# kason-huang/StreamVLN

Hardware: AMD Instinct MI355X
Metric: action-steps/sec (8-frame window, StreamVLN-Qwen-1.5) (higher is better)
Workload: dtype bf16

## Files before the change

### streamvln_amd/csrc/gemv.hip

```cpp
#include <hip/hip_ext.h>

#include <cstdlib>
#include <stdexcept>

#include "common.h"
#include "kernels.h"

namespace svln {

namespace {

typedef __attribute__((ext_vector_type(2))) __bf16 bf16x2_t;
typedef float f32x2 __attribute__((ext_vector_type(2)));
constexpr int GEMV_THREADS = 256;
constexpr int GEMV_WAVES = GEMV_THREADS / 64;


template <typename T> struct WPlain {
    using X = T;
    static constexpr int EPC = Elt<T>::PER_CHUNK;
    struct Row { const T* w; };
    using Chunk = uint4;
    using Acc = float;
    static constexpr bool X_LATE = false;
    static constexpr int ROWS_GRID_CAP = 0;
    static constexpr int KS_R = 2;
    static constexpr int KS_KW_NARROW = 4;
    static constexpr bool KS_PAIRED = true;
    SVLN_DEV static Row row(const GemvArgs& p, size_t n) { return {(const T*)p.W + n * p.ldw}; }
    SVLN_DEV static Chunk load(const Row& r, int ci) { return load_nt(r.w + (size_t)ci * EPC); }
    SVLN_DEV static Acc zero() { return 0.0f; }
    SVLN_DEV static void fma(const Chunk& w, const f32x2* x2, Acc& acc) {
        float f[EPC];
        chunk_to_f32<T>(w, f);
#pragma unroll
        for (int e = 0; e < EPC; ++e) acc = fmaf(f[e], x2[e / 2][e % 2], acc);
    }
    SVLN_DEV static float sum(Acc a) { return a; }
    SVLN_DEV static float row_scale(const GemvArgs&, size_t) { return 1.0f; }
};

struct WPacked {
    using X = bf16;
    using Acc = f32x2;
    SVLN_DEV static Acc zero() { return f32x2{0.0f, 0.0f}; }
    SVLN_DEV static float sum(Acc a) { return a[0] + a[1]; }
};

struct WE4m3 : WPacked {
    static constexpr int EPC = 16;
    struct Row { const uint8_t* w; };
    using Chunk = uint4;
    static constexpr bool X_LATE = false;
    static constexpr int ROWS_GRID_CAP = 0;
    static constexpr int KS_R = 4;
    static constexpr int KS_KW_NARROW = 4;
    static constexpr bool KS_PAIRED = false;
    SVLN_DEV static Row row(const GemvArgs& p, size_t n) { return {(const uint8_t*)p.w8 + n * p.ldw}; }
    SVLN_DEV static Chunk load(const Row& r, int ci) { return load_nt(r.w + (size_t)ci * 16); }
    SVLN_DEV static void fma(const Chunk& w, const f32x2* x2, Acc& acc) {
        const unsigned d[4] = {w.x, w.y, w.z, w.w};
#pragma unroll
        for (int q = 0; q < 4; ++q) {
            const f32x2 lo = __builtin_amdgcn_cvt_pk_f32_fp8((int)d[q], false);
            const f32x2 hi = __builtin_amdgcn_cvt_pk_f32_fp8((int)d[q], true);
            acc = __builtin_elementwise_fma(lo, x2[2 * q], acc);
            acc = __builtin_elementwise_fma(hi, x2[2 * q + 1], acc);
        }
    }
    SVLN_DEV static float row_scale(const GemvArgs& p, size_t n) { return p.scale[n]; }
};

struct WMxfp4 : WPacked {
    static constexpr int EPC = 32;
    struct Row { const uint8_t* q; const uint8_t* s; };
    struct Chunk { uint4 q; unsigned s; };
    static constexpr bool X_LATE = true;
    static constexpr int ROWS_GRID_CAP = 0;
    static constexpr int KS_R = 4;
    static constexpr int KS_KW_NARROW = 2;
    static constexpr bool KS_PAIRED = false;
    SVLN_DEV static Row row(const GemvArgs& p, size_t n) {
        return {(const uint8_t*)p.w4 + n * ((size_t)p.ldw / 2), p.e8 + n * ((size_t)p.ldw / 32)};
    }
    SVLN_DEV static Chunk load(const Row& r, int ci) { return {load_nt(r.q + (size_t)ci * 16), r.s[ci]}; }
    SVLN_DEV static void fma(const Chunk& w, const f32x2* x2, Acc& acc) {
        const unsigned d[4] = {w.q.x, w.q.y, w.q.z, w.q.w};
        const float sc = __uint_as_float(w.s << 23);
#pragma unroll
        for (int q = 0; q < 4; ++q) {
            acc = __builtin_elementwise_fma((f32x2)__builtin_amdgcn_cvt_scalef32_pk_f32_fp4(d[q], sc, 0), x2[4 * q], acc);
            acc = __builtin_elementwise_fma((f32x2)__builtin_amdgcn_cvt_scalef32_pk_f32_fp4(d[q], sc, 1), x2[4 * q + 1], acc);
            acc = __builtin_elementwise_fma((f32x2)__builtin_amdgcn_cvt_scalef32_pk_f32_fp4(d[q], sc, 2), x2[4 * q + 2], acc);
            acc = __builtin_elementwise_fma((f32x2)__builtin_amdgcn_cvt_scalef32_pk_f32_fp4(d[q], sc, 3), x2[4 * q + 3], acc);
        }
    }
    SVLN_DEV static float row_scale(const GemvArgs&, size_t) { return 1.0f; }
};

SVLN_DEV void p12_high_bytes(unsigned c, unsigned t0, unsigned t1, unsigned& ha, unsigned& hb) {
    ha = __builtin_amdgcn_perm(t1, t0, c & 0x07070707u) | ((c << 4) & 0x80808080u);
    hb = __builtin_amdgcn_perm(t1, t0, (c >> 4) & 0x07070707u) | (c & 0x80808080u);
}
SVLN_DEV uint4 p12_decode(unsigned lo0, unsigned lo1, unsigned c, unsigned t0, unsigned t1) {
    unsigned ha, hb;
    p12_high_bytes(c, t0, t1, ha, hb);
    return make_uint4(__builtin_amdgcn_perm(ha, lo0, 0x05010400u), __builtin_amdgcn_perm(ha, lo0, 0x07030602u),
                      __builtin_amdgcn_perm(hb, lo1, 0x05010400u), __builtin_amdgcn_perm(hb, lo1, 0x07030602u));
}
SVLN_DEV void p12_decode_f32(unsigned lo0, unsigned lo1, unsigned c, unsigned t0, unsigned t1, float* f) {
    unsigned ha, hb;
    p12_high_bytes(c, t0, t1, ha, hb);
    f[0] = __uint_as_float(__builtin_amdgcn_perm(ha, lo0, 0x04000C0Cu)); f[1] = __uint_as_float(__builtin_amdgcn_perm(ha, lo0, 0x05010C0Cu));
    f[2] = __uint_as_float(__builtin_amdgcn_perm(ha, lo0, 0x06020C0Cu)); f[3] = __uint_as_float(__builtin_amdgcn_perm(ha, lo0, 0x07030C0Cu));
    f[4] = __uint_as_float(__builtin_amdgcn_perm(hb, lo1, 0x04000C0Cu)); f[5] = __uint_as_float(__builtin_amdgcn_perm(hb, lo1, 0x05010C0Cu));
    f[6] = __uint_as_float(__builtin_amdgcn_perm(hb, lo1, 0x06020C0Cu)); f[7] = __uint_as_float(__builtin_amdgcn_perm(hb, lo1, 0x07030C0Cu));
}
typedef __attribute__((ext_vector_type(2))) unsigned int u32x2;
struct WP12 {
    using X = bf16;
    static constexpr int EPC = 8;
    struct Row { const uint8_t* pk; const bf16* w; unsigned t0, t1, m0, m1; };
    struct Chunk { u32x2 a, b; unsigned t0, t1; bool fb, odd; };
    using Acc = float;
    static constexpr bool X_LATE = false;
    static constexpr int ROWS_GRID_CAP = 1024;
    static constexpr int KS_R = 2;
    static constexpr int KS_KW_NARROW = 4;
    static constexpr bool KS_PAIRED = true;
    SVLN_DEV static size_t uniform(size_t v) {
        const unsigned lo = (unsigned)__builtin_amdgcn_readfirstlane((int)(unsigned)v), hi = (unsigned)__builtin_amdgcn_readfirstlane((int)(unsigned)(v >> 32));
        return ((size_t)hi << 32) | lo;
    }
    SVLN_DEV static Row row(const GemvArgs& p, size_t n) {
        const uint4 rec = *(const uint4*)((const uint8_t*)p.prec + n * 16);
        return {(const uint8_t*)p.wp + uniform(n * p12_row_bytes(p.K)), (const bf16*)p.W + uniform(n * (size_t)p.ldw),
                (unsigned)__builtin_amdgcn_readfirstlane((int)rec.x), (unsigned)__builtin_amdgcn_readfirstlane((int)rec.y),
                (unsigned)__builtin_amdgcn_readfirstlane((int)rec.z), (unsigned)__builtin_amdgcn_readfirstlane((int)rec.w)};
    }
    SVLN_DEV static Chunk load(const Row& r, int ci) {
        const int blk = __builtin_amdgcn_readfirstlane(ci >> 6);
        const unsigned l = (unsigned)ci & 63u;
        Chunk c; c.t0 = r.t0; c.t1 = r.t1; c.odd = l & 1u;
        c.fb = (((blk & 32) ? r.m1 : r.m0) >> (blk & 31)) & 1u;
        const uint8_t* wb = (const uint8_t*)r.w + (size_t)blk * 1024;
        const uint8_t* pb = r.pk + (size_t)blk * 768;
        c.a = __builtin_nontemporal_load((const u32x2*)((c.fb ? wb : pb) + (l << (c.fb ? 4 : 3))));
        c.b = __builtin_nontemporal_load((const u32x2*)((c.fb ? wb + 8 : pb + 512) + (c.fb ? l << 4 : (l >> 1) << 3)));
        return c;
    }
    SVLN_DEV static Acc zero() { return 0.0f; }
    SVLN_DEV static void fma(const Chunk& w, const f32x2* x2, Acc& acc) {
        float f[EPC];
        if (w.fb) chunk_to_f32<bf16>(make_uint4(w.a.x, w.a.y, w.b.x, w.b.y), f);
        else p12_decode_f32(w.a.x, w.a.y, w.odd ? w.b.y : w.b.x, w.t0, w.t1, f);
#pragma unroll
        for (int e = 0; e < EPC; ++e) acc = fmaf(f[e], x2[e / 2][e % 2], acc);
    }
    SVLN_DEV static float sum(Acc a) { return a; }
    SVLN_DEV static float row_scale(const GemvArgs&, size_t) { return 1.0f; }
};

template <typename X, int PLANES>
SVLN_DEV float stage_x(float* xs, const GemvArgs& p, int nch) {
    constexpr int XEPC = Elt<X>::PER_CHUNK;
    constexpr int XP = XEPC / 4, XPW = PLANES / XP;
    __shared__ float red[GEMV_WAVES];
    const X* x = (const X*)p.x;
    const X* g = (const X*)p.norm_w;
    const int tid = threadIdx.x, nxch = p.K / XEPC;
    float ss = 0.0f;
    for (int ci = tid; ci < nxch; ci += GEMV_THREADS) {
        float f[XEPC];
        chunk_to_f32<X>(*(const uint4*)(x + (size_t)ci * XEPC), f);
        if (g) {
            float gf[XEPC];
            chunk_to_f32<X>(*(const uint4*)(g + (size_t)ci * XEPC), gf);
#pragma unroll
            for (int e = 0; e < XEPC; ++e) { ss = fmaf(f[e], f[e], ss); f[e] *= gf[e]; }
        }
        const int cj = ci / XPW, p0 = (ci % XPW) * XP;
#pragma unroll
        for (int q = 0; q < XP; ++q)
            *(float4*)(xs + (size_t)(p0 + q) * nch * 4 + (size_t)cj * 4) = make_float4(f[4 * q], f[4 * q + 1], f[4 * q + 2], f[4 * q + 3]);
    }
    if (g) {
        ss = wave_sum(ss);
        if ((tid & 63) == 0) red[tid >> 6] = ss;
    }
    __syncthreads();
    if (!g) return 1.0f;
    float tot = 0.0f;
#pragma unroll
    for (int w = 0; w < GEMV_WAVES; ++w) tot += red[w];
    return rsqrtf(tot / (float)p.K + p.eps);
}

template <int PLANES>
SVLN_DEV void load_x(const float* xs, int nch, int ci, f32x2* x2) {
#pragma unroll
    for (int q = 0; q < PLANES; ++q) {
        const float4 v = *(const float4*)(xs + (size_t)q * nch * 4 + (size_t)ci * 4);
        x2[2 * q] = f32x2{v.x, v.y};
        x2[2 * q + 1] = f32x2{v.z, v.w};
    }
}
template <typename P, bool NORM>
SVLN_DEV float load_xg(const typename P::X* xg, const typename P::X* gg, int ci, f32x2* x2, float ss) {
    using X = typename P::X;
    constexpr int XEPC = Elt<X>::PER_CHUNK;
#pragma unroll
    for (int h = 0; h < P::EPC / XEPC; ++h) {
        float fh[XEPC];
        chunk_to_f32<X>(*(const uint4*)(xg + (size_t)ci * P::EPC + h * XEPC), fh);
        if (NORM) {
            float gf[XEPC];
            chunk_to_f32<X>(*(const uint4*)(gg + (size_t)ci * P::EPC + h * XEPC), gf);
#pragma unroll
            for (int e = 0; e < XEPC; ++e) { ss = fmaf(fh[e], fh[e], ss); fh[e] *= gf[e]; }
        }
#pragma unroll
        for (int e = 0; e < XEPC / 2; ++e) x2[h * (XEPC / 2) + e] = f32x2{fh[2 * e], fh[2 * e + 1]};
    }
    return ss;
}

template <typename P, int R, bool XLDS>
SVLN_DEV void dot_accum(const typename P::Row (&rows)[R], const float* xs, const typename P::X* xg, int nch, int c0, int cstep, int lane,
                        typename P::Acc (&acc)[R]) {
    constexpr int EPC = P::EPC;
    auto get_x = [&](int ci, f32x2* x2) {
        if (XLDS) load_x<EPC / 4>(xs, nch, ci, x2);
        else load_xg<P, false>(xg, nullptr, ci, x2, 0.0f);
    };
    const int stride = 64 * cstep;
    int ci = c0 + lane;
    for (; ci + stride < nch; ci += 2 * stride) {
        typename P::Chunk w0[R], w1[R];
#pragma unroll
        for (int r = 0; r < R; ++r) {
            w0[r] = P::load(rows[r], ci);
            w1[r] = P::load(rows[r], ci + stride);
        }
        f32x2 x0[EPC / 2];
        get_x(ci, x0);
        if (P::X_LATE) {
#pragma unroll
            for (int r = 0; r < R; ++r) P::fma(w0[r], x0, acc[r]);
            get_x(ci + stride, x0);
#pragma unroll
            for (int r = 0; r < R; ++r) P::fma(w1[r], x0, acc[r]);
        } else {
            f32x2 x1[EPC / 2];
            get_x(ci + stride, x1);
#pragma unroll
            for (int r = 0; r < R; ++r) {
                P::fma(w0[r], x0, acc[r]);
                P::fma(w1[r], x1, acc[r]);
            }
        }
    }
    for (; ci < nch; ci += stride) {
        typename P::Chunk w0[R];
#pragma unroll
        for (int r = 0; r < R; ++r) w0[r] = P::load(rows[r], ci);
        f32x2 x0[EPC / 2];
        get_x(ci, x0);
#pragma unroll
        for (int r = 0; r < R; ++r) P::fma(w0[r], x0, acc[r]);
    }
}

template <typename X>
SVLN_DEV void store_out(const GemvArgs& p, int n, float v) {
    if (p.bias) v += to_f32(((const X*)p.bias)[n]);
    if (p.res) v += to_f32(((const X*)p.res)[n]);
    ((X*)p.y)[n] = from_f32<X>(v);
}

template <typename P, int EPI>
__global__ __launch_bounds__(GEMV_THREADS) void gemv_rows_kernel(GemvArgs p) {
    using X = typename P::X;
    extern __shared__ __attribute__((aligned(16))) char smem_raw[];
    float* xs = (float*)smem_raw;
    const int skip = p.skip ? *p.skip : 0;
    constexpr int R = 4, OUTS = EPI == EPI_SWIGLU ? R / 2 : R;
    const int nch = p.K / P::EPC;
    const float xscale = stage_x<X, P::EPC / 4>(xs, p, nch);
    if (skip) return;
    const int lane = threadIdx.x & 63, wave = threadIdx.x >> 6;
    const int gw = blockIdx.x * GEMV_WAVES + wave, nw = gridDim.x * GEMV_WAVES;
    const int n_out = EPI == EPI_SWIGLU ? p.N >> 1 : p.N;

    constexpr HeadForm F = head_form(EPI);
    constexpr bool AMAX = epi_is_argmax(EPI), TOPK = F.topk, ENT = F.ent, LSE = F.lse, SMP = F.smp;
    static_assert(!F.tgt, "the wave-per-rows GEMV has no forced form");
    [[maybe_unused]] float tk_v = -INFINITY, tk_thr = -INFINITY;
    [[maybe_unused]] int tk_i = 0x7FFFFFFF;
    [[maybe_unused]] auto tk_insert = [&](float y, int col) {
        if (!(y > tk_thr)) return;
        const float up_v = __shfl_up(tk_v, 1, 64);
        const int up_i = __shfl_up(tk_i, 1, 64);
        if (!(tk_v >= y)) {
            const bool here = lane == 0 || up_v >= y;
            tk_v = here ? y : up_v;
            tk_i = here ? col : up_i;
        }
        tk_thr = __shfl(tk_v, TOPK_C - 1, 64);
    };
    float best = -INFINITY;
    int best_i = 0x7FFFFFFF;
    float lm = -INFINITY, ls = 0.0f;
    [[maybe_unused]] float lt = 0.0f;
    [[maybe_unused]] float best_raw = -INFINITY;
    [[maybe_unused]] int smp_stream = 0, smp_draw = 0;
    if constexpr (SMP) { smp_stream = p.smp.stream[0]; smp_draw = p.smp.draw[0] + (p.smp.count ? *p.smp.count : 0); }
    for (int n0 = gw * OUTS; n0 < n_out; n0 += nw * OUTS) {
        size_t rn[R];
#pragma unroll
        for (int u = 0; u < OUTS; ++u) {
            const int j = min(n0 + u, n_out - 1);
            if (EPI == EPI_SWIGLU) { rn[2 * u] = swiglu_gate_row(j); rn[2 * u + 1] = rn[2 * u] + 32; }
            else rn[u] = (size_t)j;
        }
        typename P::Row rows[R];
        typename P::Acc a[R];
#pragma unroll
        for (int r = 0; r < R; ++r) { rows[r] = P::row(p, rn[r]); a[r] = P::zero(); }
        dot_accum<P, R, true>(rows, xs, nullptr, nch, 0, 1, lane, a);
        float acc[R];
#pragma unroll
        for (int r = 0; r < R; ++r) acc[r] = wave_sum(P::sum(a[r])) * (P::row_scale(p, rn[r]) * xscale);
        if (EPI == EPI_SWIGLU) {
            if (lane < OUTS && n0 + lane < n_out) {
                const float gt = lane == 0 ? acc[0] : acc[2], up = lane == 0 ? acc[1] : acc[3];
                ((X*)p.y)[n0 + lane] = from_f32<X>(silu_f(gt) * up);
            }
        } else if (AMAX) {
            if (p.pen_flags) {
#pragma unroll
                for (int r = 0; r < R; ++r)
                    if (n0 + r < p.N && p.pen_flags[n0 + r]) acc[r] = acc[r] < 0.0f ? acc[r] * p.pen : acc[r] / p.pen;
            }
            if constexpr (SMP) {
                const float gq = gumbel_noise(p.smp.seed_lo, p.smp.seed_hi, smp_stream, smp_draw, n0 + (lane & 3));
#pragma unroll
                for (int r = 0; r < R; ++r) {
                    const float y = acc[r] * p.smp.inv_t, z = __fadd_rn(y, __shfl(gq, r, 64));
                    if (n0 + r < p.N) {
                        if (z > best) { best = z; best_i = n0 + r; best_raw = y; }
                        if constexpr (ENT) ent_add(y, lm, ls, lt); else lse_add(y, lm, ls);
                        if constexpr (TOPK) tk_insert(y, n0 + r);
                    }
                }
            } else {
#pragma unroll
            for (int r = 0; r < R; ++r)
                if (n0 + r < p.N && acc[r] > best) { best = acc[r]; best_i = n0 + r; }
            }
            if (LSE) {
#pragma unroll
                for (int r = 0; r < R; ++r)
                    if (n0 + r < p.N) {
                        if constexpr (ENT) ent_add(acc[r], lm, ls, lt); else lse_add(acc[r], lm, ls);
                        if constexpr (TOPK) tk_insert(acc[r], n0 + r);
                    }
            }
        } else if (lane < R && n0 + lane < p.N) {
            store_out<X>(p, n0 + lane, lane == 0 ? acc[0] : lane == 1 ? acc[1] : lane == 2 ? acc[2] : acc[3]);
        }
    }
    if (AMAX) {
        __shared__ float bv[GEMV_WAVES];
        __shared__ int bi[GEMV_WAVES];
        if constexpr (TOPK) {
            __shared__ float cv[GEMV_WAVES * TOPK_C];
            __shared__ int ci[GEMV_WAVES * TOPK_C];
            if (lane < TOPK_C) { cv[wave * TOPK_C + lane] = tk_v; ci[wave * TOPK_C + lane] = tk_i; }
            __syncthreads();
            if (threadIdx.x < GEMV_WAVES * TOPK_C) {
                const int t = threadIdx.x;
                const float v = cv[t];
                const int i = ci[t];
                int place = 0;
#pragma unroll
                for (int o = 0; o < GEMV_WAVES * TOPK_C; ++o)
                    place += cv[o] > v || (cv[o] == v && (ci[o] < i || (ci[o] == i && o < t)));
                if (place < TOPK_C) {
                    p.cand_val[(size_t)blockIdx.x * TOPK_C + place] = v;
                    p.cand_idx[(size_t)blockIdx.x * TOPK_C + place] = i;
                }
            }
        }
        if (lane == 0) { bv[wave] = best; bi[wave] = best_i; }
        if constexpr (SMP) {
            __shared__ float bs[GEMV_WAVES], bm[GEMV_WAVES], br[GEMV_WAVES];
            if (lane == 0) { bs[wave] = ls; bm[wave] = lm; br[wave] = best_raw; }
            __syncthreads();
            if (threadIdx.x == 0) {
                float v = bv[0], m = bm[0], raw = br[0]; int i = bi[0];
#pragma unroll
                for (int w = 1; w < GEMV_WAVES; ++w) {
                    if (bv[w] > v || (bv[w] == v && bi[w] < i)) { v = bv[w]; i = bi[w]; raw = br[w]; }
                    m = bm[w] > m ? bm[w] : m;
                }
                float sum = 0.0f;
#pragma unroll
                for (int w = 0; w < GEMV_WAVES; ++w) sum += lse_rescale(bs[w], bm[w], m);
                p.part_val[blockIdx.x] = v; p.part_idx[blockIdx.x] = i; p.smp.part_raw[blockIdx.x] = raw;
                p.smp.part_max[blockIdx.x] = m; p.part_sum[blockIdx.x] = sum;
            }
            if constexpr (ENT) {
                __shared__ float bt[GEMV_WAVES];
                if (lane == 0) bt[wave] = lt;
                __syncthreads();
                if (threadIdx.x == 0) {
                    float m = bm[0];
#pragma unroll
                    for (int w = 1; w < GEMV_WAVES; ++w) m = bm[w] > m ? bm[w] : m;
                    float te = 0.0f;
#pragma unroll
                    for (int w = 0; w < GEMV_WAVES; ++w) te += ent_rescale(bt[w], bs[w], bm[w], m);
                    p.part_ent[blockIdx.x] = te;
                }
            }
            return;
        }
        if constexpr (LSE) {
            __shared__ float bs[GEMV_WAVES];
            [[maybe_unused]] __shared__ float bt[ENT ? GEMV_WAVES : 1];
            if (lane == 0) bs[wave] = ls;
            if constexpr (ENT) if (lane == 0) bt[wave] = lt;
            __syncthreads();
            if (threadIdx.x == 0) {
                float v = bv[0];
#pragma unroll
                for (int w = 1; w < GEMV_WAVES; ++w) v = bv[w] > v ? bv[w] : v;
                float sum = 0.0f;
#pragma unroll
                for (int w = 0; w < GEMV_WAVES; ++w) sum += lse_rescale(bs[w], bv[w], v);
                p.part_sum[blockIdx.x] = sum;
                if constexpr (ENT) {
                    float te = 0.0f;
#pragma unroll
                    for (int w = 0; w < GEMV_WAVES; ++w) te += ent_rescale(bt[w], bs[w], bv[w], v);
                    p.part_ent[blockIdx.x] = te;
                }
            }
        } else {
            __syncthreads();
        }
        if (threadIdx.x == 0) {
            float v = bv[0]; int i = bi[0];
#pragma unroll
            for (int w = 1; w < GEMV_WAVES; ++w)
                if (bv[w] > v || (bv[w] == v && bi[w] < i)) { v = bv[w]; i = bi[w]; }
            p.part_val[blockIdx.x] = v;
            p.part_idx[blockIdx.x] = i;
        }
    }
}

template <typename P, bool NORM, int KW>
__global__ __launch_bounds__(GEMV_THREADS) void gemv_ksplit_kernel(GemvArgs p) {
    using X = typename P::X;
    constexpr int R = P::KS_R, EPC = P::EPC;
    constexpr int RG = GEMV_WAVES / KW;
    __shared__ float part[GEMV_WAVES][R + 1];
    if (p.skip && *p.skip) return;
    const int nch = p.K / EPC;
    const int lane = threadIdx.x & 63, wave = threadIdx.x >> 6;
    const int kw = RG == 1 ? wave : wave % KW, rg = RG == 1 ? 0 : wave / KW;
    const X* xg = (const X*)p.x;
    const X* gg = (const X*)p.norm_w;
    for (int b0 = blockIdx.x * RG * R; b0 < p.N; b0 += gridDim.x * RG * R) {
        const int n0 = b0 + rg * R;
        typename P::Row rows[R];
        typename P::Acc a[R];
#pragma unroll
        for (int r = 0; r < R; ++r) { rows[r] = P::row(p, (size_t)min(n0 + r, p.N - 1)); a[r] = P::zero(); }
        float ss = 0.0f;
        if (!NORM && P::KS_PAIRED) {
            dot_accum<P, R, false>(rows, nullptr, xg, nch, kw * 64, KW, lane, a);
        } else {
            for (int ci = kw * 64 + lane; ci < nch; ci += 64 * KW) {
                typename P::Chunk w[R];
#pragma unroll
                for (int r = 0; r < R; ++r) w[r] = P::load(rows[r], ci);
                __builtin_amdgcn_sched_barrier(0);
                f32x2 xf[EPC / 2];
                ss = load_xg<P, NORM>(xg, gg, ci, xf, ss);
#pragma unroll
                for (int r = 0; r < R; ++r) P::fma(w[r], xf, a[r]);
            }
        }
#pragma unroll
        for (int r = 0; r < R; ++r) asm volatile("" : "+v"(a[r]));
        float acc[R + 1];
        acc[R] = NORM ? wave_sum(ss) : 0.0f;
#pragma unroll
        for (int r = 0; r < R; ++r) acc[r] = wave_sum(P::sum(a[r]));
        if (lane == 0) {
#pragma unroll
            for (int r = 0; r <= R; ++r) part[wave][r] = acc[r];
        }
        __syncthreads();
        if (threadIdx.x < RG * R) {
            const int g2 = threadIdx.x / R, r = threadIdx.x % R, n = b0 + g2 * R + r;
            if (n < p.N) {
                float v = part[g2 * KW][r], s2 = part[g2 * KW][R];
#pragma unroll
                for (int k = 1; k < KW; ++k) { v += part[g2 * KW + k][r]; s2 += part[g2 * KW + k][R]; }
                v *= P::row_scale(p, n);
                if (NORM) v *= rsqrtf(s2 / (float)p.K + p.eps);
                store_out<X>(p, n, v);
            }
        }
        __syncthreads();
    }
}

template <typename T, int EPI, bool NORM, int B>
__global__ __launch_bounds__(GEMV_THREADS) void gemv_batched_kernel(GemvBatchArgs p) {
    constexpr int EPC = Elt<T>::PER_CHUNK, R = 4, STRIDE = 64 * GEMV_WAVES;
    __shared__ float part[GEMV_WAVES][R * B + B];
    const int nch = p.K / EPC;
    const int lane = threadIdx.x & 63, wave = threadIdx.x >> 6, tid = threadIdx.x;
    const T* W = (const T*)p.W;
    const T* xg = (const T*)p.x;
    const T* gg = (const T*)p.norm_w;
    const int n_units = EPI == EPI_SWIGLU ? p.N / R : (p.N + R - 1) / R;
    constexpr HeadForm F = head_form(EPI);
    constexpr bool AMAX = epi_is_argmax(EPI), TGT = F.tgt, TOPK = F.topk, ENT = F.ent, LSE = F.lse, SMP = F.smp;
    static_assert(!(TOPK && NORM), "EPI_*_TOPK has no fused-norm form");
    static_assert(!(ENT && NORM), "EPI_*_ENT has no fused-norm form");
    [[maybe_unused]] float tk_v[TOPK ? TOPK_C : 1];
    [[maybe_unused]] int tk_i[TOPK ? TOPK_C : 1];
    if constexpr (TOPK) {
#pragma unroll
        for (int e = 0; e < TOPK_C; ++e) { tk_v[e] = -INFINITY; tk_i[e] = 0x7FFFFFFF; }
    }
    [[maybe_unused]] auto tk_insert = [&](float y, int col) {
        if constexpr (TOPK) {
            if (!(y > tk_v[TOPK_C - 1])) return;
            bool placed = false;
#pragma unroll
            for (int e = TOPK_C - 1; e >= 1; --e) {
                if (placed) continue;
                if (tk_v[e - 1] >= y) { tk_v[e] = y; tk_i[e] = col; placed = true; }
                else { tk_v[e] = tk_v[e - 1]; tk_i[e] = tk_i[e - 1]; }
            }
            if (!placed) { tk_v[0] = y; tk_i[0] = col; }
        }
    };
    static_assert(!(SMP && NORM), "EPI_SAMPLE has no fused-norm form");
    static_assert(!(TGT && NORM), "EPI_TARGET has no fused-norm form");
    [[maybe_unused]] int my_tgt = -1;
    if constexpr (TGT) if (tid < B) my_tgt = p.tg.tgt[tid];
    float best = -INFINITY;
    int best_i = 0x7FFFFFFF;
    float lm = -INFINITY, ls = 0.0f;
    [[maybe_unused]] float lt = 0.0f;
    [[maybe_unused]] float best_raw = -INFINITY;
    [[maybe_unused]] __shared__ float gn[SMP ? R * B : 1];
    [[maybe_unused]] int smp_stream = 0, smp_draw = 0;
    if constexpr (SMP) if (tid < R * B) { smp_stream = p.smp.stream[tid % B]; smp_draw = p.smp.draw[tid % B]; }
    for (int u = blockIdx.x; u < n_units; u += gridDim.x) {
        const T* rows[R];
        int n0;
        if (EPI == EPI_SWIGLU) {
            const int j0 = u * (R / 2);
            n0 = j0;
#pragma unroll
            for (int o = 0; o < R / 2; ++o) {
                const size_t gr = swiglu_gate_row(j0 + o);
                rows[2 * o] = W + gr * p.ldw;
                rows[2 * o + 1] = W + (gr + 32) * p.ldw;
            }
        } else {
            n0 = u * R;
#pragma unroll
            for (int r = 0; r < R; ++r) rows[r] = W + (size_t)min(n0 + r, p.N - 1) * p.ldw;
        }
        float acc[R][B], ss[B];
#pragma unroll
        for (int b = 0; b < B; ++b) {
            ss[b] = 0.0f;
#pragma unroll
            for (int r = 0; r < R; ++r) acc[r][b] = 0.0f;
        }
        for (int ci = wave * 64 + lane; ci < nch; ci += STRIDE) {
            uint4 w[R], xr[B];
#pragma unroll
            for (int r = 0; r < R; ++r) w[r] = load_nt(rows[r] + (size_t)ci * EPC);
#pragma unroll
            for (int b = 0; b < B; ++b) xr[b] = *(const uint4*)(xg + (size_t)b * p.ldx + (size_t)ci * EPC);
            if (sizeof(T) == 2 && !NORM) {
#pragma unroll
                for (int b = 0; b < B; ++b) {
                    const unsigned xw[4] = {xr[b].x, xr[b].y, xr[b].z, xr[b].w};
#pragma unroll
                    for (int r = 0; r < R; ++r) {
                        const unsigned ww[4] = {w[r].x, w[r].y, w[r].z, w[r].w};
#pragma unroll
                        for (int q = 0; q < 4; ++q)
                            acc[r][b] = __builtin_amdgcn_fdot2_f32_bf16(__builtin_bit_cast(bf16x2_t, ww[q]), __builtin_bit_cast(bf16x2_t, xw[q]),
                                                                        acc[r][b], false);
                    }
                }
            } else {
                float gf[EPC];
                if (NORM) chunk_to_f32<T>(*(const uint4*)(gg + (size_t)ci * EPC), gf);
                float wf[R][EPC];
#pragma unroll
                for (int r = 0; r < R; ++r) chunk_to_f32<T>(w[r], wf[r]);
#pragma unroll
                for (int b = 0; b < B; ++b) {
                    float xf[EPC];
                    chunk_to_f32<T>(xr[b], xf);
                    if (NORM) {
#pragma unroll
                        for (int e = 0; e < EPC; ++e) { ss[b] = fmaf(xf[e], xf[e], ss[b]); xf[e] *= gf[e]; }
                    }
#pragma unroll
                    for (int r = 0; r < R; ++r)
#pragma unroll
                        for (int e = 0; e < EPC; ++e) acc[r][b] = fmaf(wf[r][e], xf[e], acc[r][b]);
                }
            }
        }
#pragma unroll
        for (int b = 0; b < B; ++b) {
            if (NORM) ss[b] = wave_sum(ss[b]);
#pragma unroll
            for (int r = 0; r < R; ++r) acc[r][b] = wave_sum(acc[r][b]);
        }
        if constexpr (SMP) if (tid < R * B) gn[tid] = gumbel_noise(p.smp.seed_lo, p.smp.seed_hi, smp_stream, smp_draw, u * R + tid / B);
        if (lane == 0) {
#pragma unroll
            for (int b = 0; b < B; ++b) {
                part[wave][R * B + b] = ss[b];
#pragma unroll
                for (int r = 0; r < R; ++r) part[wave][r * B + b] = acc[r][b];
            }
        }
        __syncthreads();
        auto total = [&](int k) { return part[0][k] + part[1][k] + part[2][k] + part[3][k]; };
        if (EPI == EPI_SWIGLU) {
            if (tid < (R / 2) * B) {
                const int o = tid / B, b = tid % B;
                const float sc = NORM ? rsqrtf(total(R * B + b) / (float)p.K + p.eps) : 1.0f;
                const float gt = total((2 * o) * B + b) * sc, up = total((2 * o + 1) * B + b) * sc;
                ((T*)p.y)[(size_t)b * p.ldy + n0 + o] = from_f32<T>(silu_f(gt) * up);
            }
        } else if (AMAX) {
            if (tid < B) {
                const uint8_t* fl = p.pen_flags ? p.pen_flags + (size_t)p.pen_rows[tid] * p.N : nullptr;
#pragma unroll
                for (int r = 0; r < R; ++r) {
                    float v = total(r * B + tid);
                    if (fl && n0 + r < p.N && fl[n0 + r]) v = v < 0.0f ? v * p.pen : v / p.pen;
                    if constexpr (TGT) {
                        v *= p.tg.inv_t;
                        if (n0 + r < p.N && n0 + r == my_tgt) p.tg.tgt_val[tid] = v;
                    }
                    if constexpr (SMP) {
                        const float y = v * p.smp.inv_t, z = __fadd_rn(y, gn[r * B + tid]);
                        if (n0 + r < p.N) {
                            if (z > best) { best = z; best_i = n0 + r; best_raw = y; }
                            if constexpr (ENT) ent_add(y, lm, ls, lt); else lse_add(y, lm, ls);
                            tk_insert(y, n0 + r);
                        }
                        continue;
                    }
                    if (n0 + r < p.N && v > best) { best = v; best_i = n0 + r; }
                    if constexpr (ENT) { if (n0 + r < p.N) ent_add(v, lm, ls, lt); }
                    else if (LSE && n0 + r < p.N) lse_add(NORM ? v * rsqrtf(total(R * B + tid) / (float)p.K + p.eps) : v, lm, ls);
                    if (TOPK && n0 + r < p.N) tk_insert(v, n0 + r);
                }
            }
        } else if (tid < R * B) {
            const int r = tid / B, b = tid % B, n = n0 + r;
            if (n < p.N) {
                float v = total(r * B + b);
                if (NORM) v *= rsqrtf(total(R * B + b) / (float)p.K + p.eps);
                if (p.bias) v += to_f32(((const T*)p.bias)[n]);
                if (p.res) v += to_f32(((const T*)p.res)[(size_t)b * p.ldr + n]);
                ((T*)p.y)[(size_t)b * p.ldy + n] = from_f32<T>(v);
            }
        }
        __syncthreads();
    }
    if (AMAX && tid < B) {
        p.part_val[(size_t)tid * gridDim.x + blockIdx.x] = best;
        p.part_idx[(size_t)tid * gridDim.x + blockIdx.x] = best_i;
        if constexpr (TOPK) {
#pragma unroll
            for (int e = 0; e < TOPK_C; ++e) {
                p.cand_val[((size_t)tid * gridDim.x + blockIdx.x) * TOPK_C + e] = tk_v[e];
                p.cand_idx[((size_t)tid * gridDim.x + blockIdx.x) * TOPK_C + e] = tk_i[e];
            }
        }
        if constexpr (ENT) p.part_ent[(size_t)tid * gridDim.x + blockIdx.x] = lt;
        if constexpr (SMP) {
            p.part_sum[(size_t)tid * gridDim.x + blockIdx.x] = ls;
            p.smp.part_max[(size_t)tid * gridDim.x + blockIdx.x] = lm;
            p.smp.part_raw[(size_t)tid * gridDim.x + blockIdx.x] = best_raw;
        }
        if (LSE) {
            p.part_sum[(size_t)tid * gridDim.x + blockIdx.x] = ls;
            if (NORM && blockIdx.x == 0) p.row_scale[tid] = rsqrtf((part[0][R * B + tid] + part[1][R * B + tid] + part[2][R * B + tid] + part[3][R * B + tid]) / (float)p.K + p.eps);
        }
    }
}


template <bool LSE, bool SMP = false>
__global__ __launch_bounds__(256) void argmax_final_batched_kernel(const float* pv, const int* pi, int n, int* out_tokens, const float* ps,
                                                                   float* scores, const float* rs, const float* pr = nullptr,
                                                                   const float* pm = nullptr) {
    __shared__ float sv[256];
    __shared__ int si[256];
    const float* v0 = pv + (size_t)blockIdx.x * n;
    const int* i0 = pi + (size_t)blockIdx.x * n;
    row_argmax_256(v0, i0, n, sv, si);
    if (threadIdx.x == 0) out_tokens[blockIdx.x] = si[0] == 0x7FFFFFFF ? -1 : si[0];
    if constexpr (SMP) {
        const int tok = si[0];
        const size_t o = (size_t)blockIdx.x * n;
        const SampleMerge mg = sample_merge(pi + o, pr + o, pm + o, ps + o, n, tok, sv, si);
        if (threadIdx.x == 0) scores[blockIdx.x] = tok == 0x7FFFFFFF ? __builtin_nanf("") : mg.raw - mg.V + lse_logprob(mg.S);
        return;
    }
    if (LSE) {
        const float sc = rs ? rs[blockIdx.x] : 1.0f;
        const float V = sv[0] * sc;
        const int tok = si[0];
        const float S = row_lse_sum_256(ps + (size_t)blockIdx.x * n, v0, n, sc, V, sv);
        if (threadIdx.x == 0) scores[blockIdx.x] = tok == 0x7FFFFFFF ? __builtin_nanf("") : lse_logprob(S);
    }
}

__global__ __launch_bounds__(256) void target_final_batched_kernel(const float* pv, const int* pi, const float* ps, int n, const int* tgt,
                                                                   const float* tgt_val, int* greedy_ids, float* greedy_logprobs, float* logprobs) {
    __shared__ float sv[256];
    __shared__ int si[256];
    const float* v0 = pv + (size_t)blockIdx.x * n;
    const int* i0 = pi + (size_t)blockIdx.x * n;
    row_argmax_256(v0, i0, n, sv, si);
    const float V = sv[0];
    const int tok = si[0];
    const float S = row_lse_sum_256(ps + (size_t)blockIdx.x * n, v0, n, 1.0f, V, sv);
    if (threadIdx.x == 0) {
        const float lp = lse_logprob(S), nan = __builtin_nanf("");
        greedy_ids[blockIdx.x] = tok == 0x7FFFFFFF ? -1 : tok;
        greedy_logprobs[blockIdx.x] = tok == 0x7FFFFFFF ? nan : lp;
        const int t = tgt[blockIdx.x];
        logprobs[blockIdx.x] = t < 0 || tok == 0x7FFFFFFF ? nan : -(-lp - (tgt_val[blockIdx.x] - V));
    }
}

__global__ __launch_bounds__(256) void quant_fp8_rows_kernel(const bf16* w, int ld, uint8_t* q, float* scale, int cols) {
    __shared__ float red[4];
    const size_t row = blockIdx.x;
    const bf16* wr = w + row * ld;
    float amax = 0.0f;
    for (int ci = threadIdx.x; ci < cols / 8; ci += 256) {
        float f[8];
        chunk_to_f32<bf16>(*(const uint4*)(wr + (size_t)ci * 8), f);
#pragma unroll
        for (int e = 0; e < 8; ++e) amax = fmaxf(amax, fabsf(f[e]));
    }
    amax = wave_max(amax);
    if ((threadIdx.x & 63) == 0) red[threadIdx.x >> 6] = amax;
    __syncthreads();
    amax = fmaxf(fmaxf(red[0], red[1]), fmaxf(red[2], red[3]));
    const float sc = e4m3_row_scale(amax);
    if (threadIdx.x == 0) scale[row] = sc;
    const float inv = 1.0f / sc;
    for (int ci = threadIdx.x; ci < cols / 8; ci += 256) {
        float f[8];
        chunk_to_f32<bf16>(*(const uint4*)(wr + (size_t)ci * 8), f);
#pragma unroll
        for (int e = 0; e < 8; ++e) f[e] = e4m3_clamp(f[e] * inv);
        int lo = 0, hi = 0;
        lo = __builtin_amdgcn_cvt_pk_fp8_f32(f[0], f[1], lo, false);
        lo = __builtin_amdgcn_cvt_pk_fp8_f32(f[2], f[3], lo, true);
        hi = __builtin_amdgcn_cvt_pk_fp8_f32(f[4], f[5], hi, false);
        hi = __builtin_amdgcn_cvt_pk_fp8_f32(f[6], f[7], hi, true);
        *(uint2*)(q + row * cols + (size_t)ci * 8) = make_uint2((unsigned)lo, (unsigned)hi);
    }
}

SVLN_DEV unsigned e2m1_code(float v) {
    const float a = fabsf(v);
    const unsigned c = (unsigned)(a > 0.25f) + (unsigned)(a >= 0.75f) + (unsigned)(a > 1.25f) + (unsigned)(a >= 1.75f) + (unsigned)(a > 2.5f) +
// ... 329 lines not shown
```

Measured before the change: 182.9.

## Deepen P12 GEMV load pipeline and move bf16 fallback off the hot path

The packed 12-bit weight GEMV now always issues loads from the packed stream (8+4 bytes per chunk) and only reloads from the bf16 copy when a block's fallback bit is set. That check is hoisted into a scalar test over all in-flight blocks, so the common path has no per-chunk select. A new deep_step/dot_accum_deep keeps three chunks of loads in flight per row before consuming them. Launch bounds now hint occupancy per kernel, and the row record is read through the constant address space. The added register pressure could reduce occupancy, and the fallback path now issues a dependent second load.

```diff
diff --git a/streamvln_amd/csrc/gemv.hip b/streamvln_amd/csrc/gemv.hip
--- a/streamvln_amd/csrc/gemv.hip
+++ b/streamvln_amd/csrc/gemv.hip
@@ -2,6 +2,7 @@
 
 #include <cstdlib>
 #include <stdexcept>
+#include <type_traits>
 
 #include "common.h"
 #include "kernels.h"
@@ -117,13 +118,15 @@
     f[6] = __uint_as_float(__builtin_amdgcn_perm(hb, lo1, 0x06020C0Cu)); f[7] = __uint_as_float(__builtin_amdgcn_perm(hb, lo1, 0x07030C0Cu));
 }
 typedef __attribute__((ext_vector_type(2))) unsigned int u32x2;
+typedef __attribute__((address_space(4))) const u32x4 p12_record_t;
 struct WP12 {
     using X = bf16;
     static constexpr int EPC = 8;
-    struct Row { const uint8_t* pk; const bf16* w; unsigned t0, t1, m0, m1; };
-    struct Chunk { u32x2 a, b; unsigned t0, t1; bool fb, odd; };
+    struct Row { const uint8_t* pk; const bf16* W; unsigned ldw, n, t0, t1, m0, m1; };
+    struct Chunk { u32x2 a; unsigned c; int blk; };
     using Acc = float;
-    static constexpr bool X_LATE = false;
+    static constexpr int DEPTH = 3, KS_DEPTH = 3;
+    static constexpr int ROWS_RESIDENT = 4, KS_RESIDENT = 1;
     static constexpr int ROWS_GRID_CAP = 1024;
     static constexpr int KS_R = 2;
     static constexpr int KS_KW_NARROW = 4;
@@ -133,33 +136,87 @@
         return ((size_t)hi << 32) | lo;
     }
     SVLN_DEV static Row row(const GemvArgs& p, size_t n) {
-        const uint4 rec = *(const uint4*)((const uint8_t*)p.prec + n * 16);
-        return {(const uint8_t*)p.wp + uniform(n * p12_row_bytes(p.K)), (const bf16*)p.W + uniform(n * (size_t)p.ldw),
-                (unsigned)__builtin_amdgcn_readfirstlane((int)rec.x), (unsigned)__builtin_amdgcn_readfirstlane((int)rec.y),
-                (unsigned)__builtin_amdgcn_readfirstlane((int)rec.z), (unsigned)__builtin_amdgcn_readfirstlane((int)rec.w)};
+        const u32x4 rec = *(p12_record_t*)((size_t)p.prec + uniform(n * 16));
+        return {(const uint8_t*)p.wp + uniform(n * p12_row_bytes(p.K)), (const bf16*)p.W, (unsigned)p.ldw, (unsigned)__builtin_amdgcn_readfirstlane((int)n), rec.x, rec.y, rec.z,
+                rec.w};
     }
     SVLN_DEV static Chunk load(const Row& r, int ci) {
-        const int blk = __builtin_amdgcn_readfirstlane(ci >> 6);
+        Chunk c;
+        c.blk = __builtin_amdgcn_readfirstlane(ci >> 6);
         const unsigned l = (unsigned)ci & 63u;
-        Chunk c; c.t0 = r.t0; c.t1 = r.t1; c.odd = l & 1u;
-        c.fb = (((blk & 32) ? r.m1 : r.m0) >> (blk & 31)) & 1u;
-        const uint8_t* wb = (const uint8_t*)r.w + (size_t)blk * 1024;
-        const uint8_t* pb = r.pk + (size_t)blk * 768;
-        c.a = __builtin_nontemporal_load((const u32x2*)((c.fb ? wb : pb) + (l << (c.fb ? 4 : 3))));
-        c.b = __builtin_nontemporal_load((const u32x2*)((c.fb ? wb + 8 : pb + 512) + (c.fb ? l << 4 : (l >> 1) << 3)));
+        const uint8_t* pb = r.pk + (size_t)c.blk * 768;
+        c.a = __builtin_nontemporal_load((const u32x2*)(pb + (l << 3)));
+        c.c = __builtin_nontemporal_load((const unsigned*)(pb + 512 + (l << 2)));
         return c;
     }
     SVLN_DEV static Acc zero() { return 0.0f; }
-    SVLN_DEV static void fma(const Chunk& w, const f32x2* x2, Acc& acc) {
+    SVLN_DEV static bool falls_back(const Row& r, int blk) { return (((blk & 32) ? r.m1 : r.m0) >> (blk & 31)) & 1u; }
+    template <int R> SVLN_DEV static bool all_packed(const Row (&rows)[R], unsigned long long blocks) {
+        unsigned long long hit = 0;
+#pragma unroll
+        for (int r = 0; r < R; ++r) {
+            unsigned long long m = ((unsigned long long)rows[r].m1 << 32) | rows[r].m0;
+            asm volatile("" : "+s"(m));
+            hit |= m & blocks;
+        }
+        return hit == 0;
+    }
+    SVLN_DEV static void chain(const float* f, const f32x2* x2, Acc& acc) {
+#pragma unroll
+        for (int e = 0; e < EPC; ++e) acc = fmaf(f[e], x2[e / 2][e % 2], acc);
+    }
+    SVLN_DEV static void fma(const Row& r, const Chunk& w, const f32x2* x2, Acc& acc) {
         float f[EPC];
-        if (w.fb) chunk_to_f32<bf16>(make_uint4(w.a.x, w.a.y, w.b.x, w.b.y), f);
-        else p12_decode_f32(w.a.x, w.a.y, w.odd ? w.b.y : w.b.x, w.t0, w.t1, f);
-#pragma unroll
-        for (int e = 0; e < EPC; ++e) acc = fmaf(f[e], x2[e / 2][e % 2], acc);
+        p12_decode_f32(w.a.x, w.a.y, w.c, r.t0, r.t1, f);
+        chain(f, x2, acc);
+    }
+    SVLN_DEV static void fma_checked(const Row& r, int ci, const Chunk& w, const f32x2* x2, Acc& acc) {
+        float f[EPC];
+        if (falls_back(r, w.blk)) {
+            unsigned off = ((unsigned)ci & 63u) << 4;
+            asm volatile("" : "+v"(off));
+            chunk_to_f32<bf16>(load_nt((const uint8_t*)(r.W + (size_t)r.n * r.ldw) + (size_t)w.blk * 1024 + off), f);
+        } else p12_decode_f32(w.a.x, w.a.y, w.c, r.t0, r.t1, f);
+        chain(f, x2, acc);
+        asm volatile("" : "+v"(acc));
     }
     SVLN_DEV static float sum(Acc a) { return a; }
     SVLN_DEV static float row_scale(const GemvArgs&, size_t) { return 1.0f; }
 };
+template <typename P, typename = void> struct StreamDepth { static constexpr bool OWN = false; static constexpr int ROWS = 2, KSPLIT = 2, ROWS_WG = 1, KS_WG = 1; };
+template <typename P> struct StreamDepth<P, decltype((void)P::DEPTH)> {
+    static constexpr bool OWN = true;
+    static constexpr int ROWS = P::DEPTH, KSPLIT = P::KS_DEPTH, ROWS_WG = P::ROWS_RESIDENT, KS_WG = P::KS_RESIDENT;
+};
+template <typename P, int R, int D>
+SVLN_DEV void consume(const typename P::Row (&rows)[R], int ci, int stride, const typename P::Chunk (&w)[D][R], const f32x2 (&x)[D][P::EPC / 2],
+                      typename P::Acc (&acc)[R]) {
+    if constexpr (std::is_same<P, WP12>::value) {
+        unsigned long long blocks = 0;
+#pragma unroll
+        for (int d = 0; d < D; ++d) blocks |= 1ull << w[d][0].blk;
+        __builtin_amdgcn_sched_barrier(0);
+        if (P::all_packed(rows, blocks)) {
+#pragma unroll
+            for (int r = 0; r < R; ++r) {
+#pragma unroll
+                for (int d = 0; d < D; ++d) P::fma(rows[r], w[d][r], x[d], acc[r]);
+            }
+        } else {
+#pragma unroll
+            for (int r = 0; r < R; ++r) {
+#pragma unroll
+                for (int d = 0; d < D; ++d) P::fma_checked(rows[r], ci + d * stride, w[d][r], x[d], acc[r]);
+            }
+        }
+    } else {
+#pragma unroll
+        for (int r = 0; r < R; ++r) {
+#pragma unroll
+            for (int d = 0; d < D; ++d) P::fma(w[d][r], x[d], acc[r]);
+        }
+    }
+}
 
 template <typename X, int PLANES>
 SVLN_DEV float stage_x(float* xs, const GemvArgs& p, int nch) {
@@ -271,6 +328,52 @@
     }
 }
 
+template <typename P, int R, bool XLDS, int D>
+SVLN_DEV void deep_step(const typename P::Row (&rows)[R], const float* xs, const typename P::X* xg, int nch, int ci, int stride,
+                        typename P::Acc (&acc)[R]) {
+    using X = typename P::X;
+    constexpr int EPC = P::EPC, XEPC = Elt<X>::PER_CHUNK, XH = EPC / XEPC;
+    [[maybe_unused]] uint4 raw[D][XH];
+    if constexpr (!XLDS) {
+#pragma unroll
+        for (int d = 0; d < D; ++d) {
+#pragma unroll
+            for (int h = 0; h < XH; ++h) raw[d][h] = *(const uint4*)(xg + (size_t)(ci + d * stride) * EPC + h * XEPC);
+        }
+    }
+    typename P::Chunk w[D][R];
+#pragma unroll
+    for (int r = 0; r < R; ++r) {
+#pragma unroll
+        for (int d = 0; d < D; ++d) w[d][r] = P::load(rows[r], ci + d * stride);
+    }
+    __builtin_amdgcn_sched_barrier(0);
+    f32x2 x[D][EPC / 2];
+#pragma unroll
+    for (int d = 0; d < D; ++d) {
+        if constexpr (XLDS) {
+            load_x<EPC / 4>(xs, nch, ci + d * stride, x[d]);
+        } else {
+#pragma unroll
+            for (int h = 0; h < XH; ++h) {
+                float fh[XEPC];
+                chunk_to_f32<X>(raw[d][h], fh);
+#pragma unroll
+                for (int e = 0; e < XEPC / 2; ++e) x[d][h * (XEPC / 2) + e] = f32x2{fh[2 * e], fh[2 * e + 1]};
+            }
+        }
+    }
+    consume<P, R, D>(rows, ci, stride, w, x, acc);
+}
+template <typename P, int R, bool XLDS, int D>
+SVLN_DEV void dot_accum_deep(const typename P::Row (&rows)[R], const float* xs, const typename P::X* xg, int nch, int c0, int cstep, int lane,
+                             typename P::Acc (&acc)[R]) {
+    const int stride = 64 * cstep;
+    int ci = c0 + lane;
+    for (; ci + (D - 1) * stride < nch; ci += D * stride) deep_step<P, R, XLDS, D>(rows, xs, xg, nch, ci, stride, acc);
+    for (; ci < nch; ci += stride) deep_step<P, R, XLDS, 1>(rows, xs, xg, nch, ci, stride, acc);
+}
+
 template <typename X>
 SVLN_DEV void store_out(const GemvArgs& p, int n, float v) {
     if (p.bias) v += to_f32(((const X*)p.bias)[n]);
@@ -279,7 +382,7 @@
 }
 
 template <typename P, int EPI>
-__global__ __launch_bounds__(GEMV_THREADS) void gemv_rows_kernel(GemvArgs p) {
+__global__ __launch_bounds__(GEMV_THREADS, StreamDepth<P>::ROWS_WG) void gemv_rows_kernel(GemvArgs p) {
     using X = typename P::X;
     extern __shared__ __attribute__((aligned(16))) char smem_raw[];
     float* xs = (float*)smem_raw;
@@ -327,7 +430,8 @@
         typename P::Acc a[R];
 #pragma unroll
         for (int r = 0; r < R; ++r) { rows[r] = P::row(p, rn[r]); a[r] = P::zero(); }
-        dot_accum<P, R, true>(rows, xs, nullptr, nch, 0, 1, lane, a);
+        if constexpr (!StreamDepth<P>::OWN) dot_accum<P, R, true>(rows, xs, nullptr, nch, 0, 1, lane, a);
+        else dot_accum_deep<P, R, true, StreamDepth<P>::ROWS>(rows, xs, nullptr, nch, 0, 1, lane, a);
         float acc[R];
 #pragma unroll
         for (int r = 0; r < R; ++r) acc[r] = wave_sum(P::sum(a[r])) * (P::row_scale(p, rn[r]) * xscale);
@@ -462,7 +566,7 @@
 }
 
 template <typename P, bool NORM, int KW>
-__global__ __launch_bounds__(GEMV_THREADS) void gemv_ksplit_kernel(GemvArgs p) {
+__global__ __launch_bounds__(GEMV_THREADS, StreamDepth<P>::KS_WG) void gemv_ksplit_kernel(GemvArgs p) {
     using X = typename P::X;
     constexpr int R = P::KS_R, EPC = P::EPC;
     constexpr int RG = GEMV_WAVES / KW;
@@ -481,17 +585,17 @@
         for (int r = 0; r < R; ++r) { rows[r] = P::row(p, (size_t)min(n0 + r, p.N - 1)); a[r] = P::zero(); }
         float ss = 0.0f;
         if (!NORM && P::KS_PAIRED) {
-            dot_accum<P, R, false>(rows, nullptr, xg, nch, kw * 64, KW, lane, a);
+            if constexpr (!StreamDepth<P>::OWN) dot_accum<P, R, false>(rows, nullptr, xg, nch, kw * 64, KW, lane, a);
+            else dot_accum_deep<P, R, false, StreamDepth<P>::KSPLIT>(rows, nullptr, xg, nch, kw * 64, KW, lane, a);
         } else {
             for (int ci = kw * 64 + lane; ci < nch; ci += 64 * KW) {
-                typename P::Chunk w[R];
-#pragma unroll
-                for (int r = 0; r < R; ++r) w[r] = P::load(rows[r], ci);
+                typename P::Chunk w[1][R];
+#pragma unroll
+                for (int r = 0; r < R; ++r) w[0][r] = P::load(rows[r], ci);
                 __builtin_amdgcn_sched_barrier(0);
-                f32x2 xf[EPC / 2];
-                ss = load_xg<P, NORM>(xg, gg, ci, xf, ss);
-#pragma unroll
-                for (int r = 0; r < R; ++r) P::fma(w[r], xf, a[r]);
+                f32x2 xf[1][EPC / 2];
+                ss = load_xg<P, NORM>(xg, gg, ci, xf[0], ss);
+                consume<P, R, 1>(rows, ci, 64 * KW, w, xf, a);
             }
         }
 #pragma unroll
```

Result: faster. 187.0 (median of 6 runs) (+2.3%).
